# MahdiGhafoorian/NLML_HPE

Hardware: AMD Instinct MI355X
Metric: faces_per_sec (higher is better)
Workload: dtype f16x2s

## Files before the change

nlml_hpe_amd/csrc/encoder_heads_f16x2_w8.hip:

```cpp
#include <hip/hip_runtime.h>

#include "../../include/nlml_hpe.h"
#include "abi_internal.h"
#include "ipd_norm.h"
#include "encoder_heads_f16x2_dev.h"
#include "layout.h"

#ifndef W8_D0_HI
#define W8_D0_HI 2
#endif
#ifndef W8_D0_LO
#define W8_D0_LO 2
#endif

namespace nlml {
namespace hx {

template <typename XHi, typename XLo, typename Extra>
__device__ __forceinline__ void step_w8(f32x16 (&acc)[2][2], f32x16 (&accS)[2][2], const h8 (&wcur)[2][2], const h8 (&xh)[2], h8 (&xl)[2],
                                        h8 (&wnext_hi)[2][2], const h8* __restrict__ wp_hi, h8 (&wnext_lo)[2][2], const h8* __restrict__ wp_lo,
                                        XHi xload_hi, XLo xload_lo, Extra extra) {
#pragma unroll
  for (int m = 0; m < 12; ++m) {
    const int t = m / 4, nb = (m % 4) / 2, fb = m % 2;
    if (t == 0) accS[nb][fb] = __builtin_amdgcn_mfma_f32_32x32x16_f16(wcur[nb][1], xh[fb], accS[nb][fb], 0, 0, 0);
    else if (t == 1) accS[nb][fb] = __builtin_amdgcn_mfma_f32_32x32x16_f16(wcur[nb][0], xl[fb], accS[nb][fb], 0, 0, 0);
    else acc[nb][fb] = __builtin_amdgcn_mfma_f32_32x32x16_f16(wcur[nb][0], xh[fb], acc[nb][fb], 0, 0, 0);
    __builtin_amdgcn_sched_barrier(0);
    if (m == 0) xload_hi(0);
    if (m == 1) xload_hi(1);
    if (m == 2) wnext_hi[0][0] = wp_hi[0];
    if (m == 4) wnext_lo[0][1] = wp_lo[64];
    if (m == 6) wnext_hi[1][0] = wp_hi[128];
    if (m == 8) xload_lo(0);
    if (m == 9) xload_lo(1);
    if (m == 10) wnext_lo[1][1] = wp_lo[192];
    extra(m);
    __builtin_amdgcn_sched_barrier(0);
  }
}

template <bool VEC4, bool NORM>
__device__ __forceinline__ void stage_e0_pass_w8(const Ctx& c, const Args& a, int64_t row0, int tid, int pass, int jw, int nbh,
                                                 f32x16 (&acc)[2][2], f32x16 (&accS)[2][2]) {
  constexpr int NB = 2, NFB = 2;
  constexpr int WSTEP = 4 * 2 * 64;
  const int F = a.F;
  const int nslab = (int)c.hdr.k8_e0 / XS_STEPS;

  const int srow = tid >> 3, scol = (tid & 7) * 4;
  int64_t r = row0 + srow;
  const bool live = r < a.B;
  r = live ? r : a.B - 1;
  const float* p = a.x + r * a.ldx;
  double ipd = 1.0, rcp = 1.0, ra = 0.0, rb = 0.0, rc = 0.0;
  if (NORM) {
    double x0, y0, z0;
    ipd_setup(p, ipd, rcp, x0, y0, z0);
    ipd_phase(scol % 3, x0, y0, z0, ra, rb, rc);
  }
  unsigned nzbits = 0u;

  struct Set { float v[4]; };
  auto gload = [&](int s, Set& st) {
    s = s < nslab ? s : nslab - 1;
    const int k = s * XS_COLS + scol;
    if (VEC4) {
      const int kc = k < F ? k : (NORM ? k - 12 * ((k - F + 15) / 12) : F - 4);
      const f32x4 t = *reinterpret_cast<const f32x4*>(p + kc);
#pragma unroll
      for (int e = 0; e < 4; ++e) st.v[e] = t[e];
    } else {
#pragma unroll
      for (int e = 0; e < 4; ++e) st.v[e] = p[k + e < F ? k + e : F - 1];
    }
  };
  auto lw_begin = [&](Set& st) {
#pragma unroll
    for (int e = 0; e < 4; ++e) asm volatile("" : "+v"(st.v[e]));
  };
  auto lw_norm = [&](Set& st, int q) {
    const int t = q % 3;
    const double rr = t == 0 ? ra : (t == 1 ? rb : rc);
    st.v[q] = (float)div_ipd((double)st.v[q] - rr, ipd, rcp);
  };
  auto lw_rotate = [&]() {
    const double t0 = rc; rc = rb; rb = ra; ra = t0;
  };
  typedef unsigned u2 __attribute__((ext_vector_type(2)));
  unsigned pend_hi[2], pend_lo[2];
  auto lw_split = [&](Set& st, int j, bool real_slab) {
    const unsigned m = real_slab ? 0x7fffffffu : 0u;
    nzbits |= (__float_as_uint(st.v[2 * j]) | __float_as_uint(st.v[2 * j + 1])) & m;
    split2(st.v[2 * j], st.v[2 * j + 1], pend_hi[j], pend_lo[j]);
  };
  constexpr int XW_PLANE = 64 * 64, XW_SLAB = 2 * XW_PLANE, XW_BUF = 2 * XW_SLAB, O_XW = LDS_BYTES - 2 * XW_BUF;
  static_assert(O_XW >= 16 * 512 * 16, "slabs behind the parked accumulators");
  const int wr_off = srow * 64 + ((((tid & 7) >> 1) ^ ((srow >> 2) & 3)) << 4) + 8 * (tid & 1);
  auto lw_store = [&](int slab_off, int piece) {
    char* d = c.lds + O_XW + slab_off + wr_off;
    if (piece == 0) *reinterpret_cast<u2*>(d) = u2{pend_hi[0], pend_hi[1]};
    else *reinterpret_cast<u2*>(d + XW_PLANE) = u2{pend_lo[0], pend_lo[1]};
  };
  auto lwrite = [&](int slab_off, Set& st, bool real_slab) {
    lw_begin(st);
    if (NORM) {
#pragma unroll
      for (int q = 0; q < 4; ++q) lw_norm(st, q);
      lw_rotate();
    }
#pragma unroll
    for (int j = 0; j < 2; ++j) lw_split(st, j, real_slab);
    lw_store(slab_off, 0);
    lw_store(slab_off, 1);
  };

  const int job = 4 * pass + jw;
  load_bias<NB, NFB>(acc, c.blob4 + c.hdr.b_off(ST_E0) + job * (4 * 8) + (2 * nbh) * 8, c.h);
  zero_acc<NB, NFB>(accS);
  const h8* w = c.blob8 + c.hdr.w_off(ST_E0) + (size_t)job * c.hdr.job_w16(ST_E0) + (2 * nbh * 2) * 64 + c.lane;
  auto wfrag = [&](int ks) { return w + (size_t)ks * WSTEP; };

  Set set[2];
  constexpr int R0 = 4, DH = W8_D0_HI, DL = W8_D0_LO;
  h8 wr[R0][NB][2];
  gload(0, set[0]);
  gload(1, set[1]);
  lwrite(0, set[0], true);
  lwrite(XW_SLAB, set[1], true);
  gload(2, set[0]);
  gload(3, set[1]);
#pragma unroll
  for (int d = 0; d < (DH > DL ? DH : DL); ++d)
#pragma unroll
    for (int nb = 0; nb < NB; ++nb)
#pragma unroll
      for (int pp = 0; pp < 2; ++pp)
        if (d < (pp ? DL : DH)) wr[d][nb][pp] = wfrag(d)[(nb * 2 + pp) * 64];
  __syncthreads();

  const int rd0 = c.f * 64 + ((c.h ^ ((c.f >> 2) & 3)) << 4);
  typedef __attribute__((address_space(3))) const char LdsC;
  LdsC* const xb0 = (LdsC*)(c.lds + O_XW + rd0);
  LdsC* const xb1 = (LdsC*)(c.lds + O_XW + (rd0 ^ 32));
  h8 xh[2][NFB], xl[NFB];
  auto xread = [&](LdsC* base, int t, int fb, int pp) {
    return *reinterpret_cast<const __attribute__((address_space(3))) h8*>(base + (t >> 1) * XW_SLAB + pp * XW_PLANE + fb * (32 * 64));
  };
  const int niter = nslab / 2;
#pragma unroll
  for (int fb = 0; fb < NFB; ++fb) {
    xh[0][fb] = xread(xb0, 0, fb, 0);
    xl[fb] = xread(xb0, 0, fb, 1);
  }
  int cur = 0, nxt = XW_BUF;
  for (int it = 0; it < niter; ++it) {
    const int s = 2 * it;
    LdsC* xc[2] = {xb0 + cur, xb1 + cur};
    LdsC* xn = xb0 + nxt;
    asm volatile("" : "+v"(xc[0]), "+v"(xc[1]), "+v"(xn));
#pragma unroll
    for (int t = 0; t < 4; ++t) {
      const int ks = 4 * it + t;
      if (t == 3) __syncthreads();
      step_w8(acc, accS, wr[t], xh[t & 1], xl, wr[(t + DH) % R0], wfrag(ks + DH), wr[(t + DL) % R0], wfrag(ks + DL),
              [&](int fb) { xh[(t + 1) & 1][fb] = t < 3 ? xread(xc[(t + 1) & 1], t + 1, fb, 0) : xread(xn, 0, fb, 0); },
              [&](int fb) { xl[fb] = t < 3 ? xread(xc[(t + 1) & 1], t + 1, fb, 1) : xread(xn, 0, fb, 1); },
              [&](int m) {
                if (t >= 2) return;
                Set& st = set[t & 1];
                const int j = m;
                const bool real = s + t + 2 < nslab;
                if (j == 0) lw_begin(st);
                if (NORM && j >= 1 && j < 5) lw_norm(st, j - 1);
                if (NORM && j == 5) lw_rotate();
                if (j == 6 || j == 7) lw_split(st, j - 6, real);
                if (j == 8) lw_store(nxt + t * XW_SLAB, 0);
                if (j == 9) lw_store(nxt + t * XW_SLAB, 1);
                if (j == 11) gload(s + t + 4, st);
              });
    }
    const int t0 = cur; cur = nxt; nxt = t0;
  }
  if (pass == 0 && a.valid) write_valid<8>(a.valid, nzbits, tid & 7, c.lane, live, row0 + srow);
}

#ifdef HX_STAMPS
#define W8S(i)                                                                                                          \
  do {                                                                                                                  \
    if (a.latent && c.lane == 0)                                                                                        \
      reinterpret_cast<unsigned long long*>(a.latent)[((size_t)blockIdx.x * 8 + c.wv) * 16 + (i)] = __builtin_amdgcn_s_memtime(); \
  } while (0)
#define W8S_WALL(i)                                                                                                     \
  do {                                                                                                                  \
    if (a.latent && c.lane == 0)                                                                                        \
      reinterpret_cast<unsigned long long*>(a.latent)[((size_t)blockIdx.x * 8 + c.wv) * 16 + (i)] = wall_clock64();     \
  } while (0)
#else
#define W8S(i) do { } while (0)
#define W8S_WALL(i) do { } while (0)
#endif

template <bool VEC4, bool NORM, bool TRUNK = false>
__global__ __launch_bounds__(512) void encoder_heads_f16x2_w8_kernel(Args a) {
  __shared__ __attribute__((aligned(16))) char lds[LDS_BYTES];

  const int tid = threadIdx.x;
  Ctx c;
  c.blob8 = reinterpret_cast<const h8*>(a.blob);
  c.blob4 = reinterpret_cast<const f32x4*>(a.blob);
  c.hdr = load_hdr(reinterpret_cast<const Header*>(a.blob));
  c.lds = lds;
  c.lane = tid & 63;
  c.f = c.lane & 31;
  c.h = c.lane >> 5;
  c.wv = __builtin_amdgcn_readfirstlane(tid >> 6);
  const int jw = c.wv >> 1, nbh = c.wv & 1;
  const int64_t row0 = (int64_t)blockIdx.x * TILE_FACES;

  {
    constexpr int WSTEP1 = 4 * 2 * 64;
    const h8* w1 = c.blob8 + c.hdr.w_off(ST_E1) + (size_t)jw * c.hdr.job_w16(ST_E1) + (2 * nbh * 2) * 64 + c.lane;
    const float inv0 = c.hdr.inv_scale[ST_E0];
    f32x16 acc1[2][2];
    f32x4* const park = reinterpret_cast<f32x4*>(c.lds + O_H1H) + tid;
    static_assert(16 * 512 * 16 <= 2 * P_H1H, "the parked layer-1 accumulators fit the h1 half image");
    load_bias<2, 2>(acc1, c.blob4 + c.hdr.b_off(ST_E1) + jw * (4 * 8) + (2 * nbh) * 8, c.h);
    auto park_acc1 = [&]() {
#pragma unroll
      for (int nb = 0; nb < 2; ++nb)
#pragma unroll
        for (int fb = 0; fb < 2; ++fb)
#pragma unroll
          for (int q = 0; q < 4; ++q)
            park[512 * ((nb * 2 + fb) * 4 + q)] = f32x4{acc1[nb][fb][4 * q], acc1[nb][fb][4 * q + 1], acc1[nb][fb][4 * q + 2], acc1[nb][fb][4 * q + 3]};
    };
    park_acc1();
    W8S(0);
    W8S_WALL(14);
#pragma unroll 1
    for (int pass = 0; pass < 2; ++pass) {
      {
        f32x16 acc0[2][2], acc0s[2][2];
        stage_e0_pass_w8<VEC4, NORM>(c, a, row0, tid, pass, jw, nbh, acc0, acc0s);
        add_acc<2, 2>(acc0, acc0s);
        W8S(1 + 4 * pass);
#pragma unroll
        for (int nb = 0; nb < 2; ++nb)
#pragma unroll
          for (int fb = 0; fb < 2; ++fb)
#pragma unroll
            for (int q = 0; q < 4; ++q) {
              const f32x4 t = park[512 * ((nb * 2 + fb) * 4 + q)];
              acc1[nb][fb][4 * q] = t[0]; acc1[nb][fb][4 * q + 1] = t[1]; acc1[nb][fb][4 * q + 2] = t[2]; acc1[nb][fb][4 * q + 3] = t[3];
            }
        __syncthreads();
        job_store<2, 2, ACT_RELU>(c, acc0, O_H1H, P_H1H, S_H1H, 128 * jw + 64 * nbh, 0, inv0);
      }
      __syncthreads();
      W8S(2 + 4 * pass);
      {
        f32x16 acc1s[2][2];
        zero_acc<2, 2>(acc1s);
        kloop<2, 2, 32, WSTEP1>(acc1, acc1s, w1 + (size_t)pass * 32 * WSTEP1, c.lds + O_H1H + (c.f * S_H1H + 8 * c.h) * 2, P_H1H,
                                32 * S_H1H * 2);
        add_acc<2, 2>(acc1, acc1s);
      }
      W8S(3 + 4 * pass);
      __syncthreads();
      if (pass == 0) park_acc1();
      W8S(4 + 4 * pass);
    }
    job_store<2, 2, ACT_RELU>(c, acc1, O_H2, P_H2, S_H2, 128 * jw + 64 * nbh, 0, c.hdr.inv_scale[ST_E1]);
  }
  __syncthreads();
  W8S(9);
  Ctx ct = c;
  ct.wv = c.wv & 3;
  f32x16 acc3[1][2];
  h8 wr3[ring_slots(1, 2)][1][2];
  {
    constexpr int WSTEP2 = 2 * 2 * 64;
    f32x16 acc2[1][2], acc2s[1][2];
    load_bias<1, 2>(acc2, c.blob4 + c.hdr.b_off(ST_E2) + jw * (2 * 8) + nbh * 8, c.h);
    zero_acc<1, 2>(acc2s);
    const h8* w2 = c.blob8 + c.hdr.w_off(ST_E2) + (size_t)jw * c.hdr.job_w16(ST_E2) + (nbh * 2) * 64 + c.lane;
    kloop<1, 2, 32, WSTEP2>(acc2, acc2s, w2, c.lds + O_H2 + (c.f * S_H2 + 8 * c.h) * 2, P_H2, 32 * S_H2 * 2);
    add_acc<1, 2>(acc2, acc2s);
    W8S(10);
    if constexpr (TRUNK) {
      typedef unsigned u4_ __attribute__((ext_vector_type(4)));
      u4_* const dst = reinterpret_cast<u4_*>(a.h3ws) + (size_t)blockIdx.x * (2 * 16 * 2 * 64) + c.lane;
#pragma unroll
      for (int fb = 0; fb < 2; ++fb) {
        h8 fr[2][2];
        frags_from_acc<ACT_RELU>(acc2[0][fb], c.hdr.inv_scale[ST_E2], fr);
#pragma unroll
        for (int p = 0; p < 2; ++p)
#pragma unroll
          for (int pc = 0; pc < 2; ++pc)
            dst[((fb * 16 + 4 * jw + 2 * nbh + p) * 2 + pc) * 64] = __builtin_bit_cast(u4_, fr[p][pc]);
      }
      return;
    }
    tail_pre_e3<false>(ct, acc3, wr3);
    __syncthreads();
    job_store<1, 2, ACT_RELU>(c, acc2, O_H3, P_H3, S_H3, 64 * jw + 32 * nbh, 0, c.hdr.inv_scale[ST_E2]);
  }
  __syncthreads();
  W8S(11);
  W8S_WALL(15);
  ct.helper = c.wv >= 4 ? 1 : 0;
  constexpr bool H1W8 = true;
#ifdef HX_STAMPS
  Args at = a;
  if (a.latent) at.latent = a.latent + (size_t)gridDim.x * 8 * 16 * 2;
  tail_stages<false, STRICT_INKERNEL_RESCUE_MAX, H1W8>(ct, at, row0, acc3, wr3);
#else
  tail_stages<false, STRICT_INKERNEL_RESCUE_MAX, H1W8>(ct, a, row0, acc3, wr3);
#endif
}

}

size_t tailws_workspace_bytes(int64_t B, int F) {
  if (B <= 0 || F <= 0) return 0;
  return (size_t)((B + TILE_FACES - 1) / TILE_FACES) * (2 * 16 * 2 * 1024);
}

int launch_encoder_heads_f16x2_tailws(const float* x, int64_t ldx, const float* raw, int normalize, int64_t B, int F,
                                      const void* blob, float* out, float* latent, uint8_t* valid, void* workspace,
                                      size_t ws_bytes, void* stream) {
  if (B == 0) return 0;
  if (!workspace || ws_bytes < tailws_workspace_bytes(B, F)) return fail(NLML_E_BADARG, "streamed-tail path: workspace too small");
  if (reinterpret_cast<uintptr_t>(workspace) & 15) return fail(NLML_E_BADARG, "streamed-tail path: workspace must be 16-byte aligned");
  const K2Input in = k2_input(x, ldx, raw, normalize, F);
  hx::Args a = k2_args<hx::Args>(in, B, F, blob, out, latent, valid);
  a.h3ws = workspace;
  if (!in.vec4) return fail(NLML_E_BADARG, "streamed-tail path: x must be 16-byte aligned with F and ldx multiples of 4");
  const int64_t ntiles = (B + TILE_FACES - 1) / TILE_FACES;
  const dim3 grid((unsigned)ntiles), block(512);
  hipStream_t st = reinterpret_cast<hipStream_t>(stream);
  if (a.norm) hipLaunchKernelGGL((hx::encoder_heads_f16x2_w8_kernel<true, true, true>), grid, block, 0, st, a);
  else hipLaunchKernelGGL((hx::encoder_heads_f16x2_w8_kernel<true, false, true>), grid, block, 0, st, a);
  if (int rc = hip_launch_status()) return rc;
  if (int rc = launch_tail_ws(blob, workspace, 2 * ntiles, B, out, latent, stream)) return rc;
  return launch_strict_reeval(x, ldx, raw, normalize, B, F, blob, out, latent, stream);
}

int launch_encoder_heads_f16x2_w8(const float* x, int64_t ldx, const float* raw, int normalize, int64_t B, int F,
                                  const void* blob, float* out, float* latent, uint8_t* valid, void* stream) {
  if (B == 0) return 0;
  const K2Input in = k2_input(x, ldx, raw, normalize, F);
  const hx::Args a = k2_args<hx::Args>(in, B, F, blob, out, latent, valid);
  const dim3 grid((unsigned)((B + TILE_FACES - 1) / TILE_FACES)), block(512);
  hipStream_t st = reinterpret_cast<hipStream_t>(stream);
  k2_with_variant(in, [&](auto V, auto N) {
    hipLaunchKernelGGL((hx::encoder_heads_f16x2_w8_kernel<decltype(V)::value, decltype(N)::value>), grid, block, 0, st, a);
  });
  if (int rc = hip_launch_status()) return rc;
  return launch_strict_reeval(x, ldx, raw, normalize, B, F, blob, out, latent, stream);
}

}
```

Baseline: 77.39 million.

## Split E0 pass into prologue and main loop, overlap prologue with layer-1 parking

Moves the E0 stage into a struct with separate pre() and run() phases. The prologue for the first pass (global loads, bias, weight prefetch, first slab writes) is issued up front. The second pass's prologue runs right after the layer-1 accumulators are parked, so its global-load latency overlaps with surrounding work. It also drops the initial park of the bias-only acc1, loading the bias directly in pass 0, which removes one LDS park/unpark round trip. In exchange, more state is held live across phases, which risks higher register pressure.

```diff
diff --git a/nlml_hpe_amd/csrc/encoder_heads_f16x2_w8.hip b/nlml_hpe_amd/csrc/encoder_heads_f16x2_w8.hip
--- a/nlml_hpe_amd/csrc/encoder_heads_f16x2_w8.hip
+++ b/nlml_hpe_amd/csrc/encoder_heads_f16x2_w8.hip
@@ -41,30 +41,25 @@
 }
 
 template <bool VEC4, bool NORM>
-__device__ __forceinline__ void stage_e0_pass_w8(const Ctx& c, const Args& a, int64_t row0, int tid, int pass, int jw, int nbh,
-                                                 f32x16 (&acc)[2][2], f32x16 (&accS)[2][2]) {
-  constexpr int NB = 2, NFB = 2;
-  constexpr int WSTEP = 4 * 2 * 64;
-  const int F = a.F;
-  const int nslab = (int)c.hdr.k8_e0 / XS_STEPS;
-
-  const int srow = tid >> 3, scol = (tid & 7) * 4;
-  int64_t r = row0 + srow;
-  const bool live = r < a.B;
-  r = live ? r : a.B - 1;
-  const float* p = a.x + r * a.ldx;
+struct E0Pass {
+  static constexpr int NB = 2, NFB = 2;
+  static constexpr int WSTEP = 4 * 2 * 64;
+  static constexpr int XW_PLANE = 64 * 64, XW_SLAB = 2 * XW_PLANE, XW_BUF = 2 * XW_SLAB, O_XW = LDS_BYTES - 2 * XW_BUF;
+  static_assert(O_XW >= 16 * 512 * 16, "slabs behind the parked accumulators");
+  static constexpr int R0 = 4, DH = W8_D0_HI, DL = W8_D0_LO;
+  struct Set { float v[4]; };
+  typedef unsigned u2 __attribute__((ext_vector_type(2)));
+
+  int F, nslab, scol, wr_off;
+  const float* p;
   double ipd = 1.0, rcp = 1.0, ra = 0.0, rb = 0.0, rc = 0.0;
-  if (NORM) {
-    double x0, y0, z0;
-    ipd_setup(p, ipd, rcp, x0, y0, z0);
-    ipd_phase(scol % 3, x0, y0, z0, ra, rb, rc);
-  }
   unsigned nzbits = 0u;
-
-  struct Set { float v[4]; };
-  auto gload = [&](int s, Set& st) {
-    s = s < nslab ? s : nslab - 1;
-    const int k = s * XS_COLS + scol;
+  unsigned pend_hi[2], pend_lo[2];
+  Set set[2], head[2];
+  h8 wr[R0][NB][2];
+  const h8* w;
+
+  __device__ __forceinline__ void gcols(int k, Set& st) const {
     if (VEC4) {
       const int kc = k < F ? k : (NORM ? k - 12 * ((k - F + 15) / 12) : F - 4);
       const f32x4 t = *reinterpret_cast<const f32x4*>(p + kc);
@@ -74,35 +69,34 @@
 #pragma unroll
       for (int e = 0; e < 4; ++e) st.v[e] = p[k + e < F ? k + e : F - 1];
     }
-  };
-  auto lw_begin = [&](Set& st) {
+  }
+  __device__ __forceinline__ void gload(int s, Set& st) const {
+    s = s < nslab ? s : nslab - 1;
+    gcols(s * XS_COLS + scol, st);
+  }
+  __device__ __forceinline__ void lw_begin(Set& st) const {
 #pragma unroll
     for (int e = 0; e < 4; ++e) asm volatile("" : "+v"(st.v[e]));
-  };
-  auto lw_norm = [&](Set& st, int q) {
+  }
+  __device__ __forceinline__ void lw_norm(Set& st, int q) const {
     const int t = q % 3;
     const double rr = t == 0 ? ra : (t == 1 ? rb : rc);
     st.v[q] = (float)div_ipd((double)st.v[q] - rr, ipd, rcp);
-  };
-  auto lw_rotate = [&]() {
+  }
+  __device__ __forceinline__ void lw_rotate() {
     const double t0 = rc; rc = rb; rb = ra; ra = t0;
-  };
-  typedef unsigned u2 __attribute__((ext_vector_type(2)));
-  unsigned pend_hi[2], pend_lo[2];
-  auto lw_split = [&](Set& st, int j, bool real_slab) {
+  }
+  __device__ __forceinline__ void lw_split(Set& st, int j, bool real_slab) {
     const unsigned m = real_slab ? 0x7fffffffu : 0u;
     nzbits |= (__float_as_uint(st.v[2 * j]) | __float_as_uint(st.v[2 * j + 1])) & m;
     split2(st.v[2 * j], st.v[2 * j + 1], pend_hi[j], pend_lo[j]);
-  };
-  constexpr int XW_PLANE = 64 * 64, XW_SLAB = 2 * XW_PLANE, XW_BUF = 2 * XW_SLAB, O_XW = LDS_BYTES - 2 * XW_BUF;
-  static_assert(O_XW >= 16 * 512 * 16, "slabs behind the parked accumulators");
-  const int wr_off = srow * 64 + ((((tid & 7) >> 1) ^ ((srow >> 2) & 3)) << 4) + 8 * (tid & 1);
-  auto lw_store = [&](int slab_off, int piece) {
+  }
+  __device__ __forceinline__ void lw_store(const Ctx& c, int slab_off, int piece) const {
     char* d = c.lds + O_XW + slab_off + wr_off;
     if (piece == 0) *reinterpret_cast<u2*>(d) = u2{pend_hi[0], pend_hi[1]};
     else *reinterpret_cast<u2*>(d + XW_PLANE) = u2{pend_lo[0], pend_lo[1]};
-  };
-  auto lwrite = [&](int slab_off, Set& st, bool real_slab) {
+  }
+  __device__ __forceinline__ void lwrite(const Ctx& c, int slab_off, Set& st, bool real_slab) {
     lw_begin(st);
     if (NORM) {
 #pragma unroll
@@ -111,79 +105,104 @@
     }
 #pragma unroll
     for (int j = 0; j < 2; ++j) lw_split(st, j, real_slab);
-    lw_store(slab_off, 0);
-    lw_store(slab_off, 1);
-  };
-
-  const int job = 4 * pass + jw;
-  load_bias<NB, NFB>(acc, c.blob4 + c.hdr.b_off(ST_E0) + job * (4 * 8) + (2 * nbh) * 8, c.h);
-  zero_acc<NB, NFB>(accS);
-  const h8* w = c.blob8 + c.hdr.w_off(ST_E0) + (size_t)job * c.hdr.job_w16(ST_E0) + (2 * nbh * 2) * 64 + c.lane;
-  auto wfrag = [&](int ks) { return w + (size_t)ks * WSTEP; };
-
-  Set set[2];
-  constexpr int R0 = 4, DH = W8_D0_HI, DL = W8_D0_LO;
-  h8 wr[R0][NB][2];
-  gload(0, set[0]);
-  gload(1, set[1]);
-  lwrite(0, set[0], true);
-  lwrite(XW_SLAB, set[1], true);
-  gload(2, set[0]);
-  gload(3, set[1]);
-#pragma unroll
-  for (int d = 0; d < (DH > DL ? DH : DL); ++d)
-#pragma unroll
-    for (int nb = 0; nb < NB; ++nb)
-#pragma unroll
-      for (int pp = 0; pp < 2; ++pp)
-        if (d < (pp ? DL : DH)) wr[d][nb][pp] = wfrag(d)[(nb * 2 + pp) * 64];
-  __syncthreads();
-
-  const int rd0 = c.f * 64 + ((c.h ^ ((c.f >> 2) & 3)) << 4);
-  typedef __attribute__((address_space(3))) const char LdsC;
-  LdsC* const xb0 = (LdsC*)(c.lds + O_XW + rd0);
-  LdsC* const xb1 = (LdsC*)(c.lds + O_XW + (rd0 ^ 32));
-  h8 xh[2][NFB], xl[NFB];
-  auto xread = [&](LdsC* base, int t, int fb, int pp) {
-    return *reinterpret_cast<const __attribute__((address_space(3))) h8*>(base + (t >> 1) * XW_SLAB + pp * XW_PLANE + fb * (32 * 64));
-  };
-  const int niter = nslab / 2;
-#pragma unroll
-  for (int fb = 0; fb < NFB; ++fb) {
-    xh[0][fb] = xread(xb0, 0, fb, 0);
-    xl[fb] = xread(xb0, 0, fb, 1);
-  }
-  int cur = 0, nxt = XW_BUF;
-  for (int it = 0; it < niter; ++it) {
-    const int s = 2 * it;
-    LdsC* xc[2] = {xb0 + cur, xb1 + cur};
-    LdsC* xn = xb0 + nxt;
-    asm volatile("" : "+v"(xc[0]), "+v"(xc[1]), "+v"(xn));
-#pragma unroll
-    for (int t = 0; t < 4; ++t) {
-      const int ks = 4 * it + t;
-      if (t == 3) __syncthreads();
-      step_w8(acc, accS, wr[t], xh[t & 1], xl, wr[(t + DH) % R0], wfrag(ks + DH), wr[(t + DL) % R0], wfrag(ks + DL),
-              [&](int fb) { xh[(t + 1) & 1][fb] = t < 3 ? xread(xc[(t + 1) & 1], t + 1, fb, 0) : xread(xn, 0, fb, 0); },
-              [&](int fb) { xl[fb] = t < 3 ? xread(xc[(t + 1) & 1], t + 1, fb, 1) : xread(xn, 0, fb, 1); },
-              [&](int m) {
-                if (t >= 2) return;
-                Set& st = set[t & 1];
-                const int j = m;
-                const bool real = s + t + 2 < nslab;
-                if (j == 0) lw_begin(st);
-                if (NORM && j >= 1 && j < 5) lw_norm(st, j - 1);
-                if (NORM && j == 5) lw_rotate();
-                if (j == 6 || j == 7) lw_split(st, j - 6, real);
-                if (j == 8) lw_store(nxt + t * XW_SLAB, 0);
-                if (j == 9) lw_store(nxt + t * XW_SLAB, 1);
-                if (j == 11) gload(s + t + 4, st);
-              });
-    }
-    const int t0 = cur; cur = nxt; nxt = t0;
-  }
-  if (pass == 0 && a.valid) write_valid<8>(a.valid, nzbits, tid & 7, c.lane, live, row0 + srow);
-}
+    lw_store(c, slab_off, 0);
+    lw_store(c, slab_off, 1);
+  }
+  __device__ __forceinline__ const h8* wfrag(int ks) const { return w + (size_t)ks * WSTEP; }
+  __device__ __forceinline__ void set_row(const Args& a, int64_t row0, int tid) {
+    int64_t r = row0 + (tid >> 3);
+    r = r < a.B ? r : a.B - 1;
+    p = a.x + r * a.ldx;
+  }
+  __device__ __forceinline__ void set_job(const Ctx& c, int pass, int jw, int nbh) {
+    w = c.blob8 + c.hdr.w_off(ST_E0) + (size_t)(4 * pass + jw) * c.hdr.job_w16(ST_E0) + (2 * nbh * 2) * 64 + c.lane;
+  }
+
+  __device__ __forceinline__ void pre(const Ctx& c, const Args& a, int64_t row0, int tid, int pass, int jw, int nbh, f32x16 (&acc)[2][2]) {
+    F = a.F;
+    const int srow = tid >> 3;
+    scol = (tid & 7) * 4;
+    wr_off = srow * 64 + ((((tid & 7) >> 1) ^ ((srow >> 2) & 3)) << 4) + 8 * (tid & 1);
+    set_row(a, row0, tid);
+    gcols(scol, head[0]);
+    gcols(XS_COLS + scol, head[1]);
+    gcols(2 * XS_COLS + scol, set[0]);
+    gcols(3 * XS_COLS + scol, set[1]);
+    if (NORM) {
+      double x0, y0, z0;
+      ipd_setup(p, ipd, rcp, x0, y0, z0);
+      ipd_phase(scol % 3, x0, y0, z0, ra, rb, rc);
+    }
+    nzbits = 0u;
+    nslab = (int)c.hdr.k8_e0 / XS_STEPS;
+    const int job = 4 * pass + jw;
+    load_bias<NB, NFB>(acc, c.blob4 + c.hdr.b_off(ST_E0) + job * (4 * 8) + (2 * nbh) * 8, c.h);
+    set_job(c, pass, jw, nbh);
+#pragma unroll
+    for (int d = 0; d < (DH > DL ? DH : DL); ++d)
+#pragma unroll
+      for (int nb = 0; nb < NB; ++nb)
+#pragma unroll
+        for (int pp = 0; pp < 2; ++pp)
+          if (d < (pp ? DL : DH)) wr[d][nb][pp] = wfrag(d)[(nb * 2 + pp) * 64];
+    lwrite(c, 0, head[0], true);
+    lwrite(c, XW_SLAB, head[1], true);
+  }
+
+  __device__ __forceinline__ void run(const Ctx& c, const Args& a, int64_t row0, int tid, int pass, int jw, int nbh,
+                                      f32x16 (&acc)[2][2], f32x16 (&accS)[2][2]) {
+    set_row(a, row0, tid);
+    set_job(c, pass, jw, nbh);
+    zero_acc<NB, NFB>(accS);
+    const int rd0 = c.f * 64 + ((c.h ^ ((c.f >> 2) & 3)) << 4);
+    typedef __attribute__((address_space(3))) const char LdsC;
+    LdsC* const xb0 = (LdsC*)(c.lds + O_XW + rd0);
+    LdsC* const xb1 = (LdsC*)(c.lds + O_XW + (rd0 ^ 32));
+    h8 xh[2][NFB], xl[NFB];
+    auto xread = [&](LdsC* base, int t, int fb, int pp) {
+      return *reinterpret_cast<const __attribute__((address_space(3))) h8*>(base + (t >> 1) * XW_SLAB + pp * XW_PLANE + fb * (32 * 64));
+    };
+    const int niter = nslab / 2;
+    int cur = 0, nxt = XW_BUF;
+#pragma unroll
+    for (int fb = 0; fb < NFB; ++fb) {
+      xh[0][fb] = xread(xb0 + cur, 0, fb, 0);
+      xl[fb] = xread(xb0 + cur, 0, fb, 1);
+    }
+    for (int it = 0; it < niter; ++it) {
+      const int s = 2 * it;
+      LdsC* xc[2] = {xb0 + cur, xb1 + cur};
+      LdsC* xn = xb0 + nxt;
+      asm volatile("" : "+v"(xc[0]), "+v"(xc[1]), "+v"(xn));
+#pragma unroll
+      for (int t = 0; t < 4; ++t) {
+        const int ks = 4 * it + t;
+        if (t == 3) __syncthreads();
+        step_w8(acc, accS, wr[t], xh[t & 1], xl, wr[(t + DH) % R0], wfrag(ks + DH), wr[(t + DL) % R0], wfrag(ks + DL),
+                [&](int fb) { xh[(t + 1) & 1][fb] = t < 3 ? xread(xc[(t + 1) & 1], t + 1, fb, 0) : xread(xn, 0, fb, 0); },
+                [&](int fb) { xl[fb] = t < 3 ? xread(xc[(t + 1) & 1], t + 1, fb, 1) : xread(xn, 0, fb, 1); },
+                [&](int m) {
+                  if (t >= 2) return;
+                  Set& st = set[t & 1];
+                  const int j = m;
+                  const bool real = s + t + 2 < nslab;
+                  if (j == 0) lw_begin(st);
+                  if (NORM && j >= 1 && j < 5) lw_norm(st, j - 1);
+                  if (NORM && j == 5) lw_rotate();
+                  if (j == 6 || j == 7) lw_split(st, j - 6, real);
+                  if (j == 8) lw_store(c, nxt + t * XW_SLAB, 0);
+                  if (j == 9) lw_store(c, nxt + t * XW_SLAB, 1);
+                  if (j == 11) gload(s + t + 4, st);
+                });
+      }
+      const int t0 = cur; cur = nxt; nxt = t0;
+    }
+  }
+  __device__ __forceinline__ void store_valid(const Ctx& c, const Args& a, int64_t row0, int tid) const {
+    const int64_t r = row0 + (tid >> 3);
+    write_valid<8>(a.valid, nzbits, tid & 7, c.lane, r < a.B, r);
+  }
+};
 
 #ifdef HX_STAMPS
 #define W8S(i)                                                                                                          \
@@ -225,7 +244,7 @@
     f32x16 acc1[2][2];
     f32x4* const park = reinterpret_cast<f32x4*>(c.lds + O_H1H) + tid;
     static_assert(16 * 512 * 16 <= 2 * P_H1H, "the parked layer-1 accumulators fit the h1 half image");
-    load_bias<2, 2>(acc1, c.blob4 + c.hdr.b_off(ST_E1) + jw * (4 * 8) + (2 * nbh) * 8, c.h);
+    auto bias_acc1 = [&]() { load_bias<2, 2>(acc1, c.blob4 + c.hdr.b_off(ST_E1) + jw * (4 * 8) + (2 * nbh) * 8, c.h); };
     auto park_acc1 = [&]() {
 #pragma unroll
       for (int nb = 0; nb < 2; ++nb)
@@ -235,42 +254,54 @@
           for (int q = 0; q < 4; ++q)
             park[512 * ((nb * 2 + fb) * 4 + q)] = f32x4{acc1[nb][fb][4 * q], acc1[nb][fb][4 * q + 1], acc1[nb][fb][4 * q + 2], acc1[nb][fb][4 * q + 3]};
     };
-    park_acc1();
+    auto unpark_acc1 = [&]() {
+#pragma unroll
+      for (int nb = 0; nb < 2; ++nb)
+#pragma unroll
+        for (int fb = 0; fb < 2; ++fb)
+#pragma unroll
+          for (int q = 0; q < 4; ++q) {
+            const f32x4 t = park[512 * ((nb * 2 + fb) * 4 + q)];
+            acc1[nb][fb][4 * q] = t[0]; acc1[nb][fb][4 * q + 1] = t[1]; acc1[nb][fb][4 * q + 2] = t[2]; acc1[nb][fb][4 * q + 3] = t[3];
+          }
+    };
+    E0Pass<VEC4, NORM> e0;
+    f32x16 acc0[2][2], acc0s[2][2];
     W8S(0);
     W8S_WALL(14);
+    e0.pre(c, a, row0, tid, 0, jw, nbh, acc0);
+    __syncthreads();
 #pragma unroll 1
-    for (int pass = 0; pass < 2; ++pass) {
-      {
-        f32x16 acc0[2][2], acc0s[2][2];
-        stage_e0_pass_w8<VEC4, NORM>(c, a, row0, tid, pass, jw, nbh, acc0, acc0s);
-        add_acc<2, 2>(acc0, acc0s);
-        W8S(1 + 4 * pass);
-#pragma unroll
-        for (int nb = 0; nb < 2; ++nb)
-#pragma unroll
-          for (int fb = 0; fb < 2; ++fb)
-#pragma unroll
-            for (int q = 0; q < 4; ++q) {
-              const f32x4 t = park[512 * ((nb * 2 + fb) * 4 + q)];
-              acc1[nb][fb][4 * q] = t[0]; acc1[nb][fb][4 * q + 1] = t[1]; acc1[nb][fb][4 * q + 2] = t[2]; acc1[nb][fb][4 * q + 3] = t[3];
-            }
-        __syncthreads();
-        job_store<2, 2, ACT_RELU>(c, acc0, O_H1H, P_H1H, S_H1H, 128 * jw + 64 * nbh, 0, inv0);
-      }
+    for (int pass = 0;; ++pass) {
+      Ctx cl = c;
+      int tl = tid;
+      asm volatile("" : "+v"(cl.lane), "+v"(cl.f), "+v"(cl.h), "+v"(tl));
+      e0.run(cl, a, row0, tl, pass, jw, nbh, acc0, acc0s);
+      if (pass == 0 && a.valid) e0.store_valid(cl, a, row0, tl);
+      add_acc<2, 2>(acc0, acc0s);
+      W8S(1 + 4 * pass);
+      if (pass == 0) bias_acc1();
+      else unpark_acc1();
+      __syncthreads();
+      job_store<2, 2, ACT_RELU>(cl, acc0, O_H1H, P_H1H, S_H1H, 128 * jw + 64 * nbh, 0, inv0);
       __syncthreads();
       W8S(2 + 4 * pass);
       {
         f32x16 acc1s[2][2];
         zero_acc<2, 2>(acc1s);
-        kloop<2, 2, 32, WSTEP1>(acc1, acc1s, w1 + (size_t)pass * 32 * WSTEP1, c.lds + O_H1H + (c.f * S_H1H + 8 * c.h) * 2, P_H1H,
+        kloop<2, 2, 32, WSTEP1>(acc1, acc1s, w1 + (size_t)pass * 32 * WSTEP1, cl.lds + O_H1H + (cl.f * S_H1H + 8 * cl.h) * 2, P_H1H,
                                 32 * S_H1H * 2);
         add_acc<2, 2>(acc1, acc1s);
       }
       W8S(3 + 4 * pass);
       __syncthreads();
-      if (pass == 0) park_acc1();
-      W8S(4 + 4 * pass);
-    }
+      if (pass == 1) break;
+      park_acc1();
+      W8S(4);
+      e0.pre(cl, a, row0, tl, 1, jw, nbh, acc0);
+      __syncthreads();
+    }
+    W8S(8);
     job_store<2, 2, ACT_RELU>(c, acc1, O_H2, P_H2, S_H2, 128 * jw + 64 * nbh, 0, c.hdr.inv_scale[ST_E1]);
   }
   __syncthreads();
```

Result: slower. 76.45 million (-1.2%).

## Make w8 encoder kernel persistent with one block per CU looping over tiles

Applied to the files above, without the earlier changes.

Switches the w8 encoder kernel to a grid-stride persistent form, launching at most one block per compute unit, with each block looping over face tiles. The header is loaded once per block, and the layer-1 bias load moves into the first pass instead of a park/unpark round trip. Opaque asm barriers keep pointers and lane values recomputed per tile so register pressure stays bounded. The aim is to cut per-block launch and prologue overhead, at the cost of a single block per CU, which may limit latency hiding and cause tail imbalance.

```diff
diff --git a/nlml_hpe_amd/csrc/encoder_heads_f16x2_w8.hip b/nlml_hpe_amd/csrc/encoder_heads_f16x2_w8.hip
--- a/nlml_hpe_amd/csrc/encoder_heads_f16x2_w8.hip
+++ b/nlml_hpe_amd/csrc/encoder_heads_f16x2_w8.hip
@@ -1,4 +1,6 @@
 #include <hip/hip_runtime.h>
+
+#include <atomic>
 
 #include "../../include/nlml_hpe.h"
 #include "abi_internal.h"
@@ -40,6 +42,24 @@
   }
 }
 
+#ifdef HX_STAMPS
+#define W8S_PUT(tile, i, v)                                                                                             \
+  do {                                                                                                                  \
+    if (a.latent && c.lane == 0) reinterpret_cast<unsigned long long*>(a.latent)[((size_t)(tile) * 8 + c.wv) * 16 + (i)] = (v); \
+  } while (0)
+#define W8T_PUT(tile, i, v)                                                                                             \
+  do {                                                                                                                  \
+    if (a.latent && c.lane == 0 && c.wv < 4)                                                                            \
+      reinterpret_cast<unsigned long long*>(a.latent)[(size_t)((a.B + TILE_FACES - 1) / TILE_FACES) * 8 * 16 +           \
+                                                      ((size_t)(tile) * 4 + c.wv) * 32 + (i)] = (v);                    \
+  } while (0)
+#else
+#define W8S_PUT(tile, i, v) do { } while (0)
+#define W8T_PUT(tile, i, v) do { } while (0)
+#endif
+#define W8S(i) W8S_PUT(tile, i, __builtin_amdgcn_s_memtime())
+#define W8S_WALL(i) W8S_PUT(tile, i, wall_clock64())
+
 template <bool VEC4, bool NORM>
 __device__ __forceinline__ void stage_e0_pass_w8(const Ctx& c, const Args& a, int64_t row0, int tid, int pass, int jw, int nbh,
                                                  f32x16 (&acc)[2][2], f32x16 (&accS)[2][2]) {
@@ -138,6 +158,7 @@
       for (int pp = 0; pp < 2; ++pp)
         if (d < (pp ? DL : DH)) wr[d][nb][pp] = wfrag(d)[(nb * 2 + pp) * 64];
   __syncthreads();
+  if (pass == 0) W8S_PUT(row0 / TILE_FACES, 13, __builtin_amdgcn_s_memtime());
 
   const int rd0 = c.f * 64 + ((c.h ^ ((c.f >> 2) & 3)) << 4);
   typedef __attribute__((address_space(3))) const char LdsC;
@@ -185,48 +206,65 @@
   if (pass == 0 && a.valid) write_valid<8>(a.valid, nzbits, tid & 7, c.lane, live, row0 + srow);
 }
 
-#ifdef HX_STAMPS
-#define W8S(i)                                                                                                          \
-  do {                                                                                                                  \
-    if (a.latent && c.lane == 0)                                                                                        \
-      reinterpret_cast<unsigned long long*>(a.latent)[((size_t)blockIdx.x * 8 + c.wv) * 16 + (i)] = __builtin_amdgcn_s_memtime(); \
-  } while (0)
-#define W8S_WALL(i)                                                                                                     \
-  do {                                                                                                                  \
-    if (a.latent && c.lane == 0)                                                                                        \
-      reinterpret_cast<unsigned long long*>(a.latent)[((size_t)blockIdx.x * 8 + c.wv) * 16 + (i)] = wall_clock64();     \
-  } while (0)
-#else
-#define W8S(i) do { } while (0)
-#define W8S_WALL(i) do { } while (0)
-#endif
+template <typename T>
+__device__ __forceinline__ T* opaque_global(T* p) {
+  auto g = (__attribute__((address_space(1))) T*)p;
+  asm volatile("" : "+s"(g));
+  return (T*)g;
+}
 
 template <bool VEC4, bool NORM, bool TRUNK = false>
-__global__ __launch_bounds__(512) void encoder_heads_f16x2_w8_kernel(Args a) {
+__global__ __launch_bounds__(512) void encoder_heads_f16x2_w8_kernel(Args a0) {
   __shared__ __attribute__((aligned(16))) char lds[LDS_BYTES];
 
-  const int tid = threadIdx.x;
-  Ctx c;
-  c.blob8 = reinterpret_cast<const h8*>(a.blob);
-  c.blob4 = reinterpret_cast<const f32x4*>(a.blob);
-  c.hdr = load_hdr(reinterpret_cast<const Header*>(a.blob));
-  c.lds = lds;
-  c.lane = tid & 63;
-  c.f = c.lane & 31;
-  c.h = c.lane >> 5;
-  c.wv = __builtin_amdgcn_readfirstlane(tid >> 6);
-  const int jw = c.wv >> 1, nbh = c.wv & 1;
-  const int64_t row0 = (int64_t)blockIdx.x * TILE_FACES;
-
+  const HdrRegs hdr = load_hdr(reinterpret_cast<const Header*>(a0.blob));
+
+  const int64_t ntiles = (a0.B + TILE_FACES - 1) / TILE_FACES;
+  for (int64_t tile = blockIdx.x; tile < ntiles; tile += gridDim.x) {
+  int tid0 = threadIdx.x;
+  asm volatile("" : "+v"(tid0));
+  Args a = a0;
+  asm volatile("" : "+s"(a.ldx), "+s"(a.B), "+s"(a.F));
+  a.x = opaque_global(a.x);
+  a.blob = opaque_global(a.blob);
+  a.out = opaque_global(a.out);
+  a.latent = opaque_global(a.latent);
+  a.valid = opaque_global(a.valid);
+  Ctx cu;
+  cu.hdr = hdr;
+  asm volatile("" : "+s"(cu.hdr.k8_e0));
+  cu.blob8 = reinterpret_cast<const h8*>(a.blob);
+  cu.blob4 = reinterpret_cast<const f32x4*>(a.blob);
+  cu.lds = lds;
+  cu.wv = __builtin_amdgcn_readfirstlane(tid0 >> 6);
+  auto lanes_of = [&](int& tid) {
+    tid = tid0;
+    asm volatile("" : "+v"(tid));
+    Ctx cx = cu;
+    cx.lane = tid & 63;
+    cx.f = cx.lane & 31;
+    cx.h = cx.lane >> 5;
+    return cx;
+  };
+  const int jw = cu.wv >> 1, nbh = cu.wv & 1;
+  constexpr int WSTEP1 = 4 * 2 * 64, WSTEP2 = 2 * 2 * 64;
+  const float inv0 = cu.hdr.inv_scale[ST_E0];
+  const int64_t row0 = tile * TILE_FACES;
   {
-    constexpr int WSTEP1 = 4 * 2 * 64;
-    const h8* w1 = c.blob8 + c.hdr.w_off(ST_E1) + (size_t)jw * c.hdr.job_w16(ST_E1) + (2 * nbh * 2) * 64 + c.lane;
-    const float inv0 = c.hdr.inv_scale[ST_E0];
+  int tid;
+  const Ctx c = lanes_of(tid);
+  W8S(12);
+  W8S(0);
+  W8S_WALL(14);
+  W8T_PUT(tile, 0, wall_clock64());
+  W8T_PUT(tile, 2, __builtin_amdgcn_s_getreg((31 << 11) | 4));
+  W8T_PUT(tile, 3, __builtin_amdgcn_s_getreg((31 << 11) | 20));
+  }
+
+  {
     f32x16 acc1[2][2];
-    f32x4* const park = reinterpret_cast<f32x4*>(c.lds + O_H1H) + tid;
     static_assert(16 * 512 * 16 <= 2 * P_H1H, "the parked layer-1 accumulators fit the h1 half image");
-    load_bias<2, 2>(acc1, c.blob4 + c.hdr.b_off(ST_E1) + jw * (4 * 8) + (2 * nbh) * 8, c.h);
-    auto park_acc1 = [&]() {
+    auto park_acc1 = [&](f32x4* park) {
 #pragma unroll
       for (int nb = 0; nb < 2; ++nb)
 #pragma unroll
@@ -235,25 +273,35 @@
           for (int q = 0; q < 4; ++q)
             park[512 * ((nb * 2 + fb) * 4 + q)] = f32x4{acc1[nb][fb][4 * q], acc1[nb][fb][4 * q + 1], acc1[nb][fb][4 * q + 2], acc1[nb][fb][4 * q + 3]};
     };
-    park_acc1();
-    W8S(0);
-    W8S_WALL(14);
 #pragma unroll 1
     for (int pass = 0; pass < 2; ++pass) {
+      f32x16 acc0[2][2];
       {
-        f32x16 acc0[2][2], acc0s[2][2];
+        f32x16 acc0s[2][2];
+        int tid;
+        const Ctx c = lanes_of(tid);
         stage_e0_pass_w8<VEC4, NORM>(c, a, row0, tid, pass, jw, nbh, acc0, acc0s);
         add_acc<2, 2>(acc0, acc0s);
+      }
+      int tid;
+      const Ctx c = lanes_of(tid);
+      const h8* const w1 = c.blob8 + c.hdr.w_off(ST_E1) + (size_t)jw * c.hdr.job_w16(ST_E1) + (2 * nbh * 2) * 64 + c.lane;
+      f32x4* const park = reinterpret_cast<f32x4*>(c.lds + O_H1H) + tid;
+      {
         W8S(1 + 4 * pass);
-#pragma unroll
-        for (int nb = 0; nb < 2; ++nb)
-#pragma unroll
-          for (int fb = 0; fb < 2; ++fb)
-#pragma unroll
-            for (int q = 0; q < 4; ++q) {
-              const f32x4 t = park[512 * ((nb * 2 + fb) * 4 + q)];
-              acc1[nb][fb][4 * q] = t[0]; acc1[nb][fb][4 * q + 1] = t[1]; acc1[nb][fb][4 * q + 2] = t[2]; acc1[nb][fb][4 * q + 3] = t[3];
-            }
+        if (pass == 0) {
+          load_bias<2, 2>(acc1, c.blob4 + c.hdr.b_off(ST_E1) + jw * (4 * 8) + (2 * nbh) * 8, c.h);
+        } else {
+#pragma unroll
+          for (int nb = 0; nb < 2; ++nb)
+#pragma unroll
+            for (int fb = 0; fb < 2; ++fb)
+#pragma unroll
+              for (int q = 0; q < 4; ++q) {
+                const f32x4 t = park[512 * ((nb * 2 + fb) * 4 + q)];
+                acc1[nb][fb][4 * q] = t[0]; acc1[nb][fb][4 * q + 1] = t[1]; acc1[nb][fb][4 * q + 2] = t[2]; acc1[nb][fb][4 * q + 3] = t[3];
+              }
+        }
         __syncthreads();
         job_store<2, 2, ACT_RELU>(c, acc0, O_H1H, P_H1H, S_H1H, 128 * jw + 64 * nbh, 0, inv0);
       }
@@ -268,23 +316,26 @@
       }
       W8S(3 + 4 * pass);
       __syncthreads();
-      if (pass == 0) park_acc1();
+      if (pass == 0) park_acc1(park);
       W8S(4 + 4 * pass);
     }
+    int tid;
+    const Ctx c = lanes_of(tid);
     job_store<2, 2, ACT_RELU>(c, acc1, O_H2, P_H2, S_H2, 128 * jw + 64 * nbh, 0, c.hdr.inv_scale[ST_E1]);
   }
   __syncthreads();
+  int tid;
+  const Ctx c = lanes_of(tid);
+  const h8* const w2 = c.blob8 + c.hdr.w_off(ST_E2) + (size_t)jw * c.hdr.job_w16(ST_E2) + (nbh * 2) * 64 + c.lane;
   W8S(9);
   Ctx ct = c;
   ct.wv = c.wv & 3;
   f32x16 acc3[1][2];
   h8 wr3[ring_slots(1, 2)][1][2];
   {
-    constexpr int WSTEP2 = 2 * 2 * 64;
     f32x16 acc2[1][2], acc2s[1][2];
     load_bias<1, 2>(acc2, c.blob4 + c.hdr.b_off(ST_E2) + jw * (2 * 8) + nbh * 8, c.h);
     zero_acc<1, 2>(acc2s);
-    const h8* w2 = c.blob8 + c.hdr.w_off(ST_E2) + (size_t)jw * c.hdr.job_w16(ST_E2) + (nbh * 2) * 64 + c.lane;
     kloop<1, 2, 32, WSTEP2>(acc2, acc2s, w2, c.lds + O_H2 + (c.f * S_H2 + 8 * c.h) * 2, P_H2, 32 * S_H2 * 2);
     add_acc<1, 2>(acc2, acc2s);
     W8S(10);
@@ -314,11 +365,13 @@
   constexpr bool H1W8 = true;
 #ifdef HX_STAMPS
   Args at = a;
-  if (a.latent) at.latent = a.latent + (size_t)gridDim.x * 8 * 16 * 2;
+  if (a.latent) at.latent = a.latent + ((size_t)ntiles * 8 * 16 + (size_t)(tile - blockIdx.x) * 4 * 32) * 2;
   tail_stages<false, STRICT_INKERNEL_RESCUE_MAX, H1W8>(ct, at, row0, acc3, wr3);
+  W8T_PUT(tile, 1, wall_clock64());
 #else
   tail_stages<false, STRICT_INKERNEL_RESCUE_MAX, H1W8>(ct, a, row0, acc3, wr3);
 #endif
+  }
 }
 
 }
@@ -348,12 +401,31 @@
   return launch_strict_reeval(x, ldx, raw, normalize, B, F, blob, out, latent, stream);
 }
 
+static int device_cu_count(int& cus) {
+  constexpr int MAX_DEVICES = 64;
+  static std::atomic<int> known[MAX_DEVICES];
+  int dev = 0;
+  hipError_t e = hipGetDevice(&dev);
+  if (e != hipSuccess) return fail((int)e, hipGetErrorString(e));
+  const bool cached = dev >= 0 && dev < MAX_DEVICES;
+  cus = cached ? known[dev].load(std::memory_order_relaxed) : 0;
+  if (cus > 0) return 0;
+  e = hipDeviceGetAttribute(&cus, hipDeviceAttributeMultiprocessorCount, dev);
+  if (e != hipSuccess) return fail((int)e, hipGetErrorString(e));
+  if (cus <= 0) return fail(NLML_E_BADARG, "device reports no compute units");
+  if (cached) known[dev].store(cus, std::memory_order_relaxed);
+  return 0;
+}
+
 int launch_encoder_heads_f16x2_w8(const float* x, int64_t ldx, const float* raw, int normalize, int64_t B, int F,
                                   const void* blob, float* out, float* latent, uint8_t* valid, void* stream) {
   if (B == 0) return 0;
   const K2Input in = k2_input(x, ldx, raw, normalize, F);
   const hx::Args a = k2_args<hx::Args>(in, B, F, blob, out, latent, valid);
-  const dim3 grid((unsigned)((B + TILE_FACES - 1) / TILE_FACES)), block(512);
+  int cus = 0;
+  if (int rc = device_cu_count(cus)) return rc;
+  const int64_t ntiles = (B + TILE_FACES - 1) / TILE_FACES;
+  const dim3 grid((unsigned)(ntiles < cus ? ntiles : cus)), block(512);
   hipStream_t st = reinterpret_cast<hipStream_t>(stream);
   k2_with_variant(in, [&](auto V, auto N) {
     hipLaunchKernelGGL((hx::encoder_heads_f16x2_w8_kernel<decltype(V)::value, decltype(N)::value>), grid, block, 0, st, a);
```

Result: no change. 80.71 million before, 80.90 million after (median of 6 runs) (+0.2%).
